# xcyan/neurips18_hierchical_image_manipulation

Hardware: AMD Instinct MI355X
Metric: mask2image train images/sec at 512x256 bs=8 (higher is better)
Workload: dtype f32; 1 GPU; C2: mask2image Cityscapes-shaped 512x256, GlobalGenerator ngf64/4down/9blocks (182.6M params) + 3-scale PatchGAN + VGG19 loss (synthetic weights), full train step G+D Adam, fp32; global_batch=8, per_gpu_batch=8, parallelism=dp1

## Files before the change

### include/him.h

```cpp
#ifndef HIM_H_
#define HIM_H_

#include <stddef.h>
#include <stdint.h>

#ifdef __cplusplus
extern "C" {
#endif

#define HIM_OK 0
#define HIM_E_INVALID (-1)
#define HIM_E_WORKSPACE (-2)
#define HIM_E_LAUNCH (-3)
#define HIM_E_UNSUPPORTED (-4)

#define HIM_ACT_NONE 0
#define HIM_ACT_RELU 1
#define HIM_ACT_LRELU 2
#define HIM_ACT_TANH 3
#define HIM_ACT_SIGMOID 4

#define HIM_PAD_ZERO 0
#define HIM_PAD_REFLECT 1

// ... 11 lines not shown
#define HIM_TILE_128x64 7

#define HIM_ALGO_NO_SPLITK (1u << 0)
#define HIM_ALGO_NO_DFOLD (1u << 1)
#define HIM_ALGO_WINO_PADDED_DGRAD (1u << 2)
#define HIM_ALGO_NO_SMALL_WIN (1u << 3)
#define HIM_ALGO_NO_FEWOUT_TILED (1u << 4)
#define HIM_ALGO_NO_FEWIN_TILED (1u << 5)
#define HIM_ALGO_NO_FEWCH_MFMA (1u << 6)
#define HIM_ALGO_GENERIC_CONV (1u << 7)
#define HIM_ALGO_NO_RESBLOCK_FUSED (1u << 8)
#define HIM_ALGO_NO_BGEMM (1u << 10)
#define HIM_ALGO_NO_ONEHOT_RLE (1u << 11)
#define HIM_ALGO_NO_FEWIN_FOLD (1u << 12)
#define HIM_ALGO_NO_FEWIN_REFLECT (1u << 14)
#define HIM_ALGO_NO_WINO_FUSED2 (1u << 15)
#define HIM_ALGO_NO_BGEMM_PERSISTENT (1u << 16)
#define HIM_ALGO_WINO4_TRAIN_FWD (1u << 13)
#define HIM_ALGO_FROZEN_WEIGHTS (1u << 9)

typedef struct HimAlgo {
  int wino_min_c;
  int wino_fused_min_c;
  int wino_fused_max_c;
  int wino4_min_c;
  int ksplit_max;
  int tile_wb, tile_nb;
  int wino_tblock;
  int wgrad_splits;
  unsigned disable;
  int wino_fused_chunk;
  int wgrad_tile;
} HimAlgo;
void him_algo_resolve(const HimAlgo* in, HimAlgo* out);
void him_algo_from_env(HimAlgo* a);

typedef struct HimConv2d {
  int B, Cin, H, W;
  int Cout, KH, KW;
  int stride, pad;
  int pad_mode;
  int OH, OW;
  int act;
  float slope;
  HimAlgo algo;
} HimConv2d;

size_t him_conv2d_fwd_ws(const HimConv2d* d);
int him_conv2d_fwd(const HimConv2d* d, const float* x, const float* w, const float* bias, float* y, void* ws,
                   size_t ws_bytes, void* stream);
size_t him_conv2d_bwd_data_ws(const HimConv2d* d);
int him_conv2d_bwd_data(const HimConv2d* d, const float* dy, const float* w, float* dx, void* ws,
                        size_t ws_bytes, void* stream);
size_t him_conv2d_bwd_weight_ws(const HimConv2d* d);
int him_conv2d_bwd_weight(const HimConv2d* d, const float* x, const float* dy, float* dw, float* dbias,
                          int accumulate, void* ws, size_t ws_bytes, void* stream);

typedef struct HimDeconv2d {
  int B, Cin, H, W;
  int Cout, KH, KW;
  int stride, pad, out_pad;
  int OH, OW;
  int act;
  float slope;
  HimAlgo algo;
} HimDeconv2d;
size_t him_deconv2d_fwd_ws(const HimDeconv2d* d);
int him_deconv2d_fwd(const HimDeconv2d* d, const float* x, const float* w, const float* bias, float* y,
                     void* ws, size_t ws_bytes, void* stream);
size_t him_deconv2d_bwd_data_ws(const HimDeconv2d* d);
int him_deconv2d_bwd_data(const HimDeconv2d* d, const float* dy, const float* w, float* dx, void* ws,
                          size_t ws_bytes, void* stream);
size_t him_deconv2d_bwd_weight_ws(const HimDeconv2d* d);
int him_deconv2d_bwd_weight(const HimDeconv2d* d, const float* x, const float* dy, float* dw, float* dbias,
                            int accumulate, void* ws, size_t ws_bytes, void* stream);
int him_conv2d_bwd_weight_plan(const HimConv2d* d, int* family, size_t* need_bytes, int* splits, int* tile_m, int* tile_n);
int him_deconv2d_bwd_weight_plan(const HimDeconv2d* d, int* family, size_t* need_bytes, int* splits, int* tile_m, int* tile_n);

size_t him_batchnorm_ws(int C);
int him_batchnorm_fwd(const float* x, const float* residual, const float* gamma, const float* beta, float* run_mean,
                      float* run_var, float* y, float* save_mean, float* save_rstd, int B, int C, int hw, float eps,
                      float momentum, int training, int act, float slope, void* ws, size_t ws_bytes, void* stream);
int him_batchnorm_bwd(const float* x, const float* gamma, const float* beta, const float* save_mean,
                      const float* save_rstd, const float* dy, float* dx, float* dgamma, float* dbeta, int B, int C,
                      int hw, int training, int act, float slope, int accumulate, void* ws, size_t ws_bytes,
                      void* stream);
int him_act_fwd(const float* x, float* y, size_t n, int act, float slope, void* stream);
int him_upsample2_fwd(const float* x, float* y, int planes, int H, int W, int align_corners, void* stream);
int him_upsample2_bwd(const float* dy, float* dx, int planes, int H, int W, int align_corners, void* stream);
int him_resize_compose(const float* comb_prob, const float* obj_prob, int C, int h, int w, const float* label,
                       const float* mask_out, int cls, int background, void* dst, int H, int W, int align_corners,
                       void* stream);
int him_logsoftmax_fwd(const float* x, float* y, int B, int C, int hw, void* stream);
int him_logsoftmax_bwd(const float* y, const float* dy, float* dx, int B, int C, int hw, void* stream);
int him_gate_comb_fwd(const float* ctx, const float* p, const float* obj, float* out, int B, int C, int hw, void* stream);
int him_gate_comb_bwd(const float* ctx, const float* p, const float* obj, const float* dout, float* dctx, float* dp,
                      float* dobj, int B, int C, int hw, void* stream);
size_t him_mask_loss_ws(void);
int him_masked_nll_fwd(const float* logp, const float* label, const float* mask, float* out2, int B, int C, int hw,
                       void* ws, size_t ws_bytes, void* stream);
int him_masked_nll_bwd(const float* label, const float* mask, const float* g, const float* count, float* dlogp, int B,
                       int C, int hw, void* stream);
int him_bce_mean_fwd(const float* p, const float* t, size_t n, float* out, void* ws, size_t ws_bytes, void* stream);
int him_bce_mean_bwd(const float* p, const float* t, size_t n, const float* g, float* dp, void* stream);
int him_space_to_batch(const float* x, float* y, int B, int C, int H, int W, int d, int inverse, void* stream);
int him_lr_control(const float* loss_d_real, const float* loss_d_fake, float margin, float* out2, void* stream);
int him_class_mask(const float* mask, const float* cls, float* dst, int B, int NC, int Ctot, int c0, int hw, void* stream);

size_t him_conv2d_onehot_fwd_ws(const HimConv2d* d, int n_onehot);
int him_conv2d_onehot_fwd(const HimConv2d* d, const float* label, int n_onehot, const float* x, const float* w,
// ... 258 lines not shown
```

### neurips18_hierchical_image_manipulation_amd/_cabi.py

```python
import ctypes as C
import os

_HERE = os.path.dirname(os.path.abspath(__file__))
LIB_PATH = os.path.join(_HERE, 'lib', 'libhim_hip.so')

c_float_p = C.c_void_p
c_int, c_size_t, c_float, c_void_p, c_double = C.c_int, C.c_size_t, C.c_float, C.c_void_p, C.c_double


class HimAlgo(C.Structure):
    _fields_ = [(n, c_int) for n in ('wino_min_c', 'wino_fused_min_c', 'wino_fused_max_c', 'wino4_min_c', 'ksplit_max',
                                     'tile_wb', 'tile_nb', 'wino_tblock', 'wgrad_splits')] + \
               [('disable', C.c_uint), ('wino_fused_chunk', c_int), ('wgrad_tile', c_int)]

    def as_dict(self):
        return {n: int(getattr(self, n)) for n, _ in self._fields_ if n != 'reserved'}


ALGO_NO_SPLITK, ALGO_NO_DFOLD, ALGO_WINO_PADDED_DGRAD, ALGO_NO_SMALL_WIN, ALGO_NO_FEWOUT_TILED, ALGO_NO_FEWIN_TILED, \
    ALGO_NO_FEWCH_MFMA, ALGO_GENERIC_CONV, ALGO_NO_RESBLOCK_FUSED, ALGO_FROZEN_WEIGHTS, ALGO_NO_BGEMM, ALGO_NO_ONEHOT_RLE = (1 << i for i in range(12))
ALGO_NO_FEWIN_FOLD = 1 << 12
ALGO_WINO4_TRAIN_FWD = 1 << 13
ALGO_NO_FEWIN_REFLECT = 1 << 14
ALGO_NO_WINO_FUSED2 = 1 << 15
ALGO_NO_BGEMM_PERSISTENT = 1 << 16
ONEHOT_PART_IDS, ONEHOT_PART_DENSE = 1, 2
TILE_DEFAULT, TILE_128x128, TILE_128x128_8W, TILE_128x256, TILE_64x128, TILE_64x64, TILE_MIXED, TILE_128x64 = range(8)


class HimConv2d(C.Structure):
    _fields_ = [(n, c_int) for n in ('B', 'Cin', 'H', 'W', 'Cout', 'KH', 'KW', 'stride', 'pad', 'pad_mode',
                                     'OH', 'OW', 'act')] + [('slope', c_float), ('algo', HimAlgo)]


class HimDeconv2d(C.Structure):
    _fields_ = [(n, c_int) for n in ('B', 'Cin', 'H', 'W', 'Cout', 'KH', 'KW', 'stride', 'pad', 'out_pad',
                                     'OH', 'OW', 'act')] + [('slope', c_float), ('algo', HimAlgo)]


class HimResBlock(C.Structure):
    _fields_ = [(n, c_int) for n in ('B', 'C', 'H', 'W')] + [('eps', c_float), ('algo', HimAlgo)]


ACT_NONE, ACT_RELU, ACT_LRELU, ACT_TANH, ACT_SIGMOID = 0, 1, 2, 3, 4
PAD_ZERO, PAD_REFLECT = 0, 1

P = c_void_p
_CONV, _DECONV, _RESB, _ALGO = C.POINTER(HimConv2d), C.POINTER(HimDeconv2d), C.POINTER(HimResBlock), C.POINTER(HimAlgo)

_SIGS = {
    'him_version': (C.c_char_p, []),
    'him_arch': (C.c_char_p, []),
    'him_last_error': (C.c_char_p, []),
    'him_conv2d_fwd_ws': (c_size_t, [_CONV]),
    'him_conv2d_fwd': (c_int, [_CONV, P, P, P, P, P, c_size_t, P]),
    'him_conv2d_bwd_data_ws': (c_size_t, [_CONV]),
    'him_conv2d_bwd_data': (c_int, [_CONV, P, P, P, P, c_size_t, P]),
    'him_conv2d_bwd_weight_ws': (c_size_t, [_CONV]),
    'him_conv2d_bwd_weight': (c_int, [_CONV, P, P, P, P, c_int, P, c_size_t, P]),
    'him_deconv2d_fwd_ws': (c_size_t, [_DECONV]),
    'him_deconv2d_fwd': (c_int, [_DECONV, P, P, P, P, P, c_size_t, P]),
    'him_deconv2d_bwd_data_ws': (c_size_t, [_DECONV]),
    'him_deconv2d_bwd_data': (c_int, [_DECONV, P, P, P, P, c_size_t, P]),
    'him_deconv2d_bwd_weight_ws': (c_size_t, [_DECONV]),
    'him_deconv2d_bwd_weight': (c_int, [_DECONV, P, P, P, P, c_int, P, c_size_t, P]),
    'him_conv2d_bwd_weight_plan': (c_int, [_CONV, C.POINTER(c_int), C.POINTER(c_size_t)] + [C.POINTER(c_int)] * 3),
    'him_deconv2d_bwd_weight_plan': (c_int, [_DECONV, C.POINTER(c_int), C.POINTER(c_size_t)] + [C.POINTER(c_int)] * 3),
    'him_algo_resolve': (None, [_ALGO, _ALGO]),
    'him_algo_from_env': (None, [_ALGO]),
    'him_conv2d_onehot_fwd_ws': (c_size_t, [_CONV, c_int]),
    'him_conv2d_onehot_fwd': (c_int, [_CONV, P, c_int, P, P, P, P, P, c_size_t, P]),
    'him_conv2d_onehot_bwd_weight_ws': (c_size_t, [_CONV, c_int]),
    'him_conv2d_onehot_bwd_weight': (c_int, [_CONV, P, c_int, P, P, P, P, c_int, P, c_size_t, P]),
    'him_conv2d_onehot_fwd_dense': (c_int, [_CONV, P, c_int, P, P, P, P, P, c_size_t, P]),
    'him_conv2d_onehot_bwd_weight_dense': (c_int, [_CONV, P, c_int, P, P, P, P, c_int, P, c_size_t, P]),
    'him_conv2d_onehot_bwd_weight_part': (c_int, [_CONV, P, c_int, P, c_int, P, P, P, c_int, P, c_size_t, c_int, P]),
    'him_winograd_gemm': (c_int, [P, P, P, c_int, c_int, c_int, _ALGO, P]),
    'him_conv2d_panel_bytes': (c_size_t, [_CONV, c_int]),
    'him_conv2d_bwd_data_shares_fwd_panel': (C.c_uint, [_CONV]),
    'him_conv2d_panel_layout': (C.c_uint, [_CONV, c_int]),
    'him_conv2d_panel_build': (c_int, [_CONV, c_int, P, P, c_size_t, P]),
    'him_conv2d_fwd_panel': (c_int, [_CONV, P, P, P, P, P, c_size_t, P]),
    'him_conv2d_bwd_data_panel': (c_int, [_CONV, P, P, P, P, c_size_t, P]),
    'him_conv2d_bwd_data_gated': (c_int, [_CONV, P, P, P, P, P, P, c_size_t, P]),
    'him_conv2d_fwd_keep_bytes': (c_size_t, [_CONV]),
    'him_conv2d_fwd_panel_keep': (c_int, [_CONV, P, P, P, P, P, P, c_size_t, P]),
    'him_conv2d_bwd_weight_kept': (c_int, [_CONV, P, P, P, P, c_int, P, c_size_t, P]),
    'him_deconv2d_panel_bytes': (c_size_t, [_DECONV, c_int]),
    'him_deconv2d_panel_build': (c_int, [_DECONV, c_int, P, P, c_size_t, P]),
    'him_deconv2d_fwd_panel': (c_int, [_DECONV, P, P, P, P, P, c_size_t, P]),
    'him_deconv2d_bwd_data_panel': (c_int, [_DECONV, P, P, P, P, c_size_t, P]),
    'him_batchnorm_ws': (c_size_t, [c_int]),
    'him_batchnorm_fwd': (c_int, [P, P, P, P, P, P, P, P, P, c_int, c_int, c_int, c_float, c_float, c_int, c_int, c_float,
                                  P, c_size_t, P]),
    'him_batchnorm_bwd': (c_int, [P, P, P, P, P, P, P, P, P, c_int, c_int, c_int, c_int, c_int, c_float, c_int, P,
                                  c_size_t, P]),
    'him_act_fwd': (c_int, [P, P, c_size_t, c_int, c_float, P]),
    'him_upsample2_fwd': (c_int, [P, P, c_int, c_int, c_int, c_int, P]),
    'him_upsample2_bwd': (c_int, [P, P, c_int, c_int, c_int, c_int, P]),
    'him_resize_compose': (c_int, [P, P, c_int, c_int, c_int, P, P, c_int, c_int, P, c_int, c_int, c_int, P]),
# ... 164 lines not shown
```

### neurips18_hierchical_image_manipulation_amd/csrc/him_conv.hip

```cpp
#include <stdlib.h>

#include <algorithm>
#include <type_traits>

#include "him_common.h"

namespace him {

#include "him_gconv_fast.inc"
#include "him_wino_fused.inc"
#include "him_wino_fused2.inc"
#include "him_bgemm.inc"

struct WT2Phase {
  float* out;
  int JH, JW;
  long long sh, sw, base;
  long long total;
};
struct WT2P {
  const float* W;
  int M, C2, C2p;
  long long sm, sc;
  WT2Phase ph[4];
// ... 402 lines not shown
  if (reflect) hipLaunchKernelGGL((wino_input_kernel<true>), gin, dim3(tb), 0, st, src, V, gi);
  else hipLaunchKernelGGL((wino_input_kernel<false>), gin, dim3(tb), 0, st, src, V, gi);
  int rc = check_launch("wino_input");
  if (rc) return rc;
  rc = wino_batched_gemm(a, U, V, Mo, Mout, Csrc, gi.Tp, st, atrans);
  if (rc) return rc;
  WinoGeom go = gi;
  go.C = Mout;
  hipLaunchKernelGGL(wino_output_kernel, dim3(cdiv(gi.Tp, tb), Mout), dim3(tb), 0, st, (const float*)Mo, dst, bias, go,
                     act, slope);
  return check_launch("wino_output");
}

#include "him_conv_wino4.inc"

#include "him_conv_wgrad.inc"

#include "him_wgrad_fewch.inc"

enum WGradFamily { WGRAD_WINO, WGRAD_HEAD, WGRAD_STEM, WGRAD_SMALL_WIN, WGRAD_SMALL, WGRAD_FAST, WGRAD_GENERIC };
struct WGradShape {
  int M, C, B, H, W, OH, OW, KH, KW, stride, pad, pad_mode;
  int Np() const { return C * KH * KW; }
  int Kdim() const { return B * OH * OW; }
};
static WGradShape wgrad_shape(const HimConv2d* d) {
  return {d->Cout, d->Cin, d->B, d->H, d->W, d->OH, d->OW, d->KH, d->KW, d->stride, d->pad, d->pad_mode};
}
struct WGradPlan {
  HimAlgo algo;
  WGradShape s;
  WGradFamily family;
  int BM, BN;
  int splits;
  int kchunk;
  bool reduce;
  size_t need_bytes;
  size_t slab_bytes;
};
static const int SMALL_WIN_SLOTS = 256;
static int small_wgrad_slices(int C, int Kdim) {
  int s = (2048 + C - 1) / C;
  const int maxs = cdiv(Kdim, 256 * 8);
  if (s > maxs) s = maxs;
  return s < 1 ? 1 : s;
}
static bool small_win_class(int M, int KH, int KW) { return M <= 4 && KH == KW && (KH == 3 || KH == 5 || KH == 7); }
static bool small_class(int M, int KH, int KW) { return M <= 4 && KH == KW && (KH == 7 || KH == 4 || KH == 3); }
static bool wgrad_same_geom(const WGradShape& s) {
  return s.stride == 1 && s.pad == s.KH / 2 && s.OH == s.H && s.OW == s.W && s.H > s.pad && s.W > s.pad;
}
static size_t round256(size_t n) { return (n + 255) / 256 * 256; }

static WGradPlan plan_wgrad(const HimAlgo& a, const WGradShape& s, bool allow_wino) {
  WGradPlan p;
  memset(&p, 0, sizeof(p));
  p.algo = a;
  p.s = s;
  p.splits = 1;
  p.reduce = true;
  const int M = s.M, C = s.C, Kdim = s.Kdim();
  const auto slabs = [&](int n) { return (size_t)n * M * s.Np() * sizeof(float); };
  const bool head_c = fewch_class(a, M, C, s.KH, s.KW), stem_c = fewch_class(a, C, M, s.KH, s.KW);
  const bool win_c = small_win_class(M, s.KH, s.KW), small_c = small_class(M, s.KH, s.KW), fast_c = wgrad_fast_class(a, M, C);
  const int fewch_tc = head_c ? C : M, slices = small_wgrad_slices(C, Kdim), tiny_n = std::max(slices, SMALL_WIN_SLOTS);
  int gBM, gBN, fBM = 0, fBN = 0, fs = 0;
  wgrad_tile(M, &gBM, &gBN);
  int gs = wgrad_splits(M, s.Np(), Kdim, gBM, gBN);
  if (win_c && !small_c && !head_c) gs = std::min(gs, tiny_n);
  if (fast_c) wgrad_fast_cfg(a, M, C, Kdim, s.KH * s.KW, &fBM, &fBN, &fs);
  const size_t generic = gs > 1 ? slabs(gs) : 0, tiny = slabs(tiny_n);
  const bool fits31 = (unsigned long long)s.B * M * s.OH * s.OW * 4ull < (1ull << 31) &&
                      (unsigned long long)s.B * C * s.H * s.W * 4ull < (1ull << 31);
  if (allow_wino && wino_wgrad_ok(a, M, C, s.KH, s.KW, s.stride, s.pad, s.H, s.W) && s.OH == s.H && s.OW == s.W) {
    p.family = WGRAD_WINO;
    p.need_bytes = wino_wgrad_floats(s.B, M, C, s.OH, s.OW) * sizeof(float);
    p.slab_bytes = round256(p.need_bytes);
    return p;
  }
  if ((head_c || stem_c) && wgrad_same_geom(s)) {
    p.family = head_c ? WGRAD_HEAD : WGRAD_STEM;
    p.splits = std::min(fewch_geom(head_c, s.B, s.H, s.W, s.pad).ntask, FEWCH_WGS);
    p.need_bytes = fewch_need_bytes(fewch_tc, s.KH, p.splits);
  } else if (win_c && !algo_off(a, HIM_ALGO_NO_SMALL_WIN) && wgrad_same_geom(s)) {
    p.family = WGRAD_SMALL_WIN;
    p.splits = std::min(s.B * cdiv(s.W, 64) * cdiv(s.H, 64), SMALL_WIN_SLOTS);
    p.need_bytes = slabs(p.splits);
  } else if (small_c) {
    p.family = WGRAD_SMALL;
    p.splits = slices;
    p.kchunk = cdiv(Kdim, slices);
    p.need_bytes = slabs(slices);
  } else if (fast_c && s.OH * s.OW >= 4 && fits31) {
    p.family = WGRAD_FAST;
    p.BM = fBM, p.BN = fBN, p.splits = fs;
    p.kchunk = (cdiv(Kdim, fs) + 31) / 32 * 32;
    p.need_bytes = slabs(fs);
  } else {
    p.family = WGRAD_GENERIC;
    p.BM = gBM, p.BN = gBN, p.splits = gs;
    p.kchunk = (cdiv(Kdim, gs) + 31) / 32 * 32;
    p.reduce = gs > 1;
    p.need_bytes = generic;
  }
  size_t b;
  if (head_c || stem_c) b = std::max(std::max(fewch_need_bytes(fewch_tc, s.KH, FEWCH_WGS), generic), (win_c || small_c) ? tiny : 0);
  else if (win_c || small_c) b = tiny;
  else if (fast_c) b = std::max(slabs(fs), generic);
  else b = generic;
  p.slab_bytes = round256(b);
  return p;
}

static int wgrad_finish(const WGradPlan& p, const char* what, const float* part, float* dw, int accumulate, hipStream_t st) {
  const int rc = check_launch(what);
  if (rc || !p.reduce) return rc;
  if (p.family == WGRAD_FAST) {
    hipLaunchKernelGGL(wgrad_finish_kernel, dim3(p.s.C / 64, p.s.M), dim3(256), 0, st, part, dw, p.s.M, p.s.C, p.s.KH * p.s.KW,
                       p.splits, accumulate);
    return check_launch("wgrad_finish");
  }
  const long long n = (long long)p.s.M * p.s.Np();
  hipLaunchKernelGGL(slab_reduce_kernel, dim3(std::min<long long>(cdiv(n, 256), 4096)), dim3(256), 0, st, part, dw, n, p.splits,
                     accumulate);
  return check_launch("slab_reduce");
}

static int run_wgrad(const WGradPlan& pl, const float* dy, const float* x, float* dw, int accumulate, void* ws, size_t ws_bytes,
                     hipStream_t st, const float* kept_v = nullptr) {
  if (pl.need_bytes && (ws_bytes < pl.need_bytes || !ws))
// ... 45 lines not shown
    case WGRAD_HEAD:
    case WGRAD_STEM:
      return run_wgrad_fewch(pl.family == WGRAD_HEAD, dy, x, dw, M, C, B, H, W, KH, s.pad, s.pad_mode, pl.splits, accumulate, ws, st);
    case WGRAD_SMALL_WIN: {
      const int nsx = cdiv(W, 64), rows_per = 64, nyc = cdiv(H, rows_per), ntasks = B * nsx * nyc;
      const dim3 grid(pl.splits, cdiv(C, 4));
#define HIM_SWK(MMv, KSv)                                                                                         \
  if (M == MMv && KH == KSv) {                                                                                    \
    constexpr int TRv = (MMv * KSv * KSv > 90) ? (KSv + 1) / 2 : KSv;   \
    const dim3 gridz(grid.x, grid.y, cdiv(KSv, TRv));                                                             \
    if (refl) hipLaunchKernelGGL((wgrad_small_win_kernel<MMv, KSv, TRv, true>), gridz, block, 0, st, p, nsx, nyc, rows_per, ntasks); \
    else hipLaunchKernelGGL((wgrad_small_win_kernel<MMv, KSv, TRv, false>), gridz, block, 0, st, p, nsx, nyc, rows_per, ntasks);     \
  }
      HIM_SWK(1, 3) HIM_SWK(2, 3) HIM_SWK(3, 3) HIM_SWK(4, 3)
      HIM_SWK(1, 5) HIM_SWK(2, 5) HIM_SWK(3, 5) HIM_SWK(4, 5)
      HIM_SWK(1, 7) HIM_SWK(2, 7) HIM_SWK(3, 7) HIM_SWK(4, 7)
#undef HIM_SWK
      return wgrad_finish(pl, "wgrad_small_win", (const float*)ws, dw, accumulate, st);
    }
    case WGRAD_SMALL: {
      const dim3 grid(C, pl.splits);
#define HIM_WS(MMv, TJv)                                                                             \
  if (M == MMv && KH == TJv) {                                                                       \
    if (refl) hipLaunchKernelGGL((wgrad_small_kernel<MMv, TJv, true>), grid, block, 0, st, p);        \
    else hipLaunchKernelGGL((wgrad_small_kernel<MMv, TJv, false>), grid, block, 0, st, p);            \
  }
      HIM_WS(1, 7) HIM_WS(2, 7) HIM_WS(3, 7) HIM_WS(4, 7)
      HIM_WS(1, 4) HIM_WS(2, 4) HIM_WS(3, 4) HIM_WS(4, 4)
      HIM_WS(1, 3) HIM_WS(2, 3) HIM_WS(3, 3) HIM_WS(4, 3)
#undef HIM_WS
      return wgrad_finish(pl, "wgrad_small", (const float*)ws, dw, accumulate, st);
    }
    case WGRAD_FAST: {
      const dim3 grid(p.Np / pl.BN, cdiv(M, pl.BM), pl.splits);
#define HIM_WF(TMv, TNv)                                                                              \
  {                                                                                                   \
    if ((s.OH * s.OW) % 4 == 0) {                                                                     \
      if (refl) hipLaunchKernelGGL((wgrad_fast_kernel<TMv, TNv, true, true>), grid, block, 0, st, p);  \
      else hipLaunchKernelGGL((wgrad_fast_kernel<TMv, TNv, false, true>), grid, block, 0, st, p);      \
    } else {                                                                                          \
      if (refl) hipLaunchKernelGGL((wgrad_fast_kernel<TMv, TNv, true, false>), grid, block, 0, st, p); \
      else hipLaunchKernelGGL((wgrad_fast_kernel<TMv, TNv, false, false>), grid, block, 0, st, p);     \
    }                                                                                                 \
  }
      if (pl.BM == 128 && pl.BN == 128) HIM_WF(2, 2)
      else if (pl.BM == 128) HIM_WF(2, 1)
      else if (pl.BN == 128) HIM_WF(1, 2)
      else HIM_WF(1, 1)
#undef HIM_WF
      return wgrad_finish(pl, "wgrad_fast", (const float*)ws, dw, accumulate, st);
    }
    case WGRAD_GENERIC: {
      const dim3 grid(cdiv(p.Np, pl.BN), cdiv(M, pl.BM), pl.splits);
      if (pl.BM == 128) {
        if (refl) hipLaunchKernelGGL((wgrad_kernel<2, 2, 2, 2, true>), grid, block, 0, st, p);
        else hipLaunchKernelGGL((wgrad_kernel<2, 2, 2, 2, false>), grid, block, 0, st, p);
      } else if (pl.BM == 64) {
        if (refl) hipLaunchKernelGGL((wgrad_kernel<1, 4, 2, 1, true>), grid, block, 0, st, p);
        else hipLaunchKernelGGL((wgrad_kernel<1, 4, 2, 1, false>), grid, block, 0, st, p);
      } else {
        if (refl) hipLaunchKernelGGL((wgrad_kernel<1, 4, 1, 1, true>), grid, block, 0, st, p);
        else hipLaunchKernelGGL((wgrad_kernel<1, 4, 1, 1, false>), grid, block, 0, st, p);
      }
      return wgrad_finish(pl, "wgrad", (const float*)ws, dw, accumulate, st);
    }
  }
// ... 501 lines not shown
  c->OH = t->H;
  c->OW = t->W;
  c->act = HIM_ACT_NONE;
  c->slope = 0.f;
  c->algo = t->algo;
  if ((c->H + 2 * c->pad - c->KH) / c->stride + 1 != c->OH || (c->W + 2 * c->pad - c->KW) / c->stride + 1 != c->OW)
    return fail(HIM_E_UNSUPPORTED, "deconv2d: output_padding %d not representable", t->out_pad);
  return check_conv(c);
}

}

using namespace him;

#include "him_resblock.inc"

extern "C" {

void him_algo_resolve(const HimAlgo* in, HimAlgo* out) {
  if (!out) return;
  HimAlgo z;
  memset(&z, 0, sizeof(z));
  const HimAlgo& a = in ? *in : z;
  HimAlgo r = a;
  r.wino_min_c = algo_wino_min_c(a);
  r.wino_fused_min_c = algo_wino_fused_min_c(a);
  r.wino_fused_max_c = algo_wino_fused_max_c(a);
  r.wino4_min_c = algo_wino4_min_c(a);
  r.ksplit_max = algo_off(a, HIM_ALGO_NO_SPLITK) ? 1 : algo_ksplit_max(a);
  r.tile_wb = a.tile_wb == HIM_TILE_DEFAULT ? HIM_TILE_64x128 : a.tile_wb;
  r.tile_nb = a.tile_nb == HIM_TILE_DEFAULT ? HIM_TILE_64x128 : a.tile_nb;
  r.wino_tblock = algo_tblock(a);
  r.wino_fused_chunk = algo_wino_fused_chunk(a);
  r.wgrad_tile = (a.wgrad_tile == 1 || a.wgrad_tile == 2) ? a.wgrad_tile : 0;
  *out = r;
}

void him_algo_from_env(HimAlgo* a) {
  if (!a) return;
  memset(a, 0, sizeof(*a));
  auto geti = [](const char* k, int dflt) { const char* e = getenv(k); return e ? atoi(e) : dflt; };
  a->wino_min_c = getenv("HIM_NO_WINOGRAD") ? -1 : geti("HIM_WINO_MIN_C", 0);
  a->wino_fused_min_c = getenv("HIM_NO_WINO_FUSED") ? -1 : geti("HIM_WINO_FUSED_MIN_C", 0);
  a->wino_fused_max_c = geti("HIM_WINO_FUSED_MAX_C", 0);
  a->wino4_min_c = getenv("HIM_NO_WINO4") ? -1 : geti("HIM_WINO4_MIN_C", 0);
  a->ksplit_max = geti("HIM_KSPLIT_MAX", 0);
  const int tile_all = geti("HIM_GCONV_TILE", 0);
  a->tile_wb = geti("HIM_GCONV_TILE_WB", tile_all);
  a->tile_nb = geti("HIM_GCONV_TILE_NB", tile_all);
  a->wino_tblock = geti("HIM_WINO_TBLOCK", 0);
  a->wgrad_splits = geti("HIM_WGRAD_SPLITS", 0);
  a->wino_fused_chunk = geti("HIM_WINO_FUSED_CHUNK", 0);
  a->wgrad_tile = geti("HIM_WGRAD_TILE", 0);
  const struct { const char* k; unsigned bit; } flags[] = {
      {"HIM_NO_SPLITK", HIM_ALGO_NO_SPLITK},           {"HIM_NO_DFOLD", HIM_ALGO_NO_DFOLD},
      {"HIM_WINO_PADDED_DGRAD", HIM_ALGO_WINO_PADDED_DGRAD}, {"HIM_NO_SMALL_WIN", HIM_ALGO_NO_SMALL_WIN},
      {"HIM_NO_FEWOUT_TILED", HIM_ALGO_NO_FEWOUT_TILED}, {"HIM_NO_FEWIN_TILED", HIM_ALGO_NO_FEWIN_TILED},
      {"HIM_NO_FEWCH_MFMA", HIM_ALGO_NO_FEWCH_MFMA},   {"HIM_GENERIC_CONV", HIM_ALGO_GENERIC_CONV},
      {"HIM_NO_RESBLOCK_FUSED", HIM_ALGO_NO_RESBLOCK_FUSED}, {"HIM_NO_BGEMM", HIM_ALGO_NO_BGEMM},
      {"HIM_NO_ONEHOT_RLE", HIM_ALGO_NO_ONEHOT_RLE},   {"HIM_NO_FEWIN_FOLD", HIM_ALGO_NO_FEWIN_FOLD},
      {"HIM_WINO4_TRAIN_FWD", HIM_ALGO_WINO4_TRAIN_FWD}, {"HIM_NO_FEWIN_REFLECT", HIM_ALGO_NO_FEWIN_REFLECT},
      {"HIM_NO_WINO_FUSED2", HIM_ALGO_NO_WINO_FUSED2}, {"HIM_NO_BGEMM_PERSISTENT", HIM_ALGO_NO_BGEMM_PERSISTENT}};
  for (const auto& f : flags)
    if (getenv(f.k)) a->disable |= f.bit;
}

int him_winograd_gemm(const float* a, const float* b, float* c, int M, int K, int N, const HimAlgo* algo, void* stream) {
  if (!a || !b || !c || M <= 4 || K < 16 || (K % 16) || N <= 0 || (N % 128))
    return fail(HIM_E_INVALID, "winograd gemm: need M > 4, K %% 16 == 0, N %% 128 == 0 (got %d, %d, %d)", M, K, N);
  if ((long long)16 * K * N >= (1ll << 31) || (long long)16 * M * N >= (1ll << 31))
    return fail(HIM_E_UNSUPPORTED, "winograd gemm: operand larger than 2^31 elements");
  HimAlgo z;
  memset(&z, 0, sizeof(z));
  return wino_batched_gemm(algo ? *algo : z, a, b, c, M, K, N, (hipStream_t)stream);
}

size_t him_conv2d_fwd_ws(const HimConv2d* d) { return d ? plan_fprop(d).ws_bytes : 0; }

int him_conv2d_fwd(const HimConv2d* d, const float* x, const float* w, const float* bias, float* y, void* ws,
                   size_t ws_bytes, void* stream) {
  int rc = check_conv(d);
  if (rc) return rc;
  return run_fprop(d, x, w, bias, y, ws, ws_bytes, (hipStream_t)stream);
}

int him_conv2d_in_act_fused(const HimConv2d* d) { return (d && !check_conv(d) && plan_fprop(d).in_act_slab) ? 1 : 0; }
// ... 106 lines not shown
}
static int conv_bwd_weight(const HimConv2d* d, const float* x, const float* keep, const float* dy, float* dw, float* dbias,
                           int accumulate, void* ws, size_t ws_bytes, hipStream_t st) {
  const WGradPlan p = plan_wgrad(d->algo, wgrad_shape(d), true);
  if (dw) {
    int rc = run_wgrad(p, dy, x, dw, accumulate, ws, ws_bytes, st, keep);
    if (rc) return rc;
  }
  if (!dbias) return HIM_OK;
  return run_bias_grad_behind(dy, dbias, d->B, d->Cout, d->OH * d->OW, accumulate, ws, ws_bytes, p.slab_bytes, st);
}
int him_conv2d_bwd_weight_kept(const HimConv2d* d, const float* keep, const float* dy, float* dw, float* dbias, int accumulate,
                               void* ws, size_t ws_bytes, void* stream) {
  int rc = check_conv(d);
  if (rc) return rc;
  if (!keep || !fwd_keep_ok(d)) return fail(HIM_E_INVALID, "conv bwd_weight_kept: no kept transform for this descriptor");
  return conv_bwd_weight(d, nullptr, keep, dy, dw, dbias, accumulate, ws, ws_bytes, (hipStream_t)stream);
}

size_t him_conv2d_bwd_weight_ws(const HimConv2d* d) {
  return d ? plan_wgrad(d->algo, wgrad_shape(d), true).slab_bytes + bias_ws_bytes(d->Cout) : 0;
}
static int report_wgrad_plan(const WGradPlan& p, int* family, size_t* need_bytes, int* splits, int* tile_m, int* tile_n) {
  if (family) *family = p.family;
  if (need_bytes) *need_bytes = p.need_bytes;
  if (splits) *splits = p.splits;
  if (tile_m) *tile_m = p.BM;
  if (tile_n) *tile_n = p.BN;
  return HIM_OK;
}
int him_conv2d_bwd_weight_plan(const HimConv2d* d, int* family, size_t* need_bytes, int* splits, int* tile_m, int* tile_n) {
  const int rc = check_conv(d);
  return rc ? rc : report_wgrad_plan(plan_wgrad(d->algo, wgrad_shape(d), true), family, need_bytes, splits, tile_m, tile_n);
}

int him_conv2d_bwd_weight(const HimConv2d* d, const float* x, const float* dy, float* dw, float* dbias,
                          int accumulate, void* ws, size_t ws_bytes, void* stream) {
  int rc = check_conv(d);
  if (rc) return rc;
  return conv_bwd_weight(d, x, nullptr, dy, dw, dbias, accumulate, ws, ws_bytes, (hipStream_t)stream);
}

size_t him_conv2d_onehot_fwd_ws(const HimConv2d* d, int n_onehot) {
  return (d && !check_conv(d) && onehot_ok(d, n_onehot)) ? onehot_fwd_ws_bytes(d, n_onehot) : 0;
}

static int onehot_fwd_impl(const HimConv2d* d, const float* label, int n_onehot, const float* x, bool x_dense, const float* w,
                           const float* bias, float* y, void* ws, size_t ws_bytes, void* stream) {
  int rc = check_conv(d);
  if (rc) return rc;
  if (!onehot_ok(d, n_onehot))
    return fail(HIM_E_UNSUPPORTED, "onehot conv: needs an odd 'same' stride-1 kernel or 4x4 stride 2 zero-padded, Cout %% 16 == 0");
  if (!ws || ws_bytes < onehot_fwd_ws_bytes(d, n_onehot)) return fail(HIM_E_WORKSPACE, "onehot conv fwd: ws too small");
  hipStream_t st = (hipStream_t)stream;
  const int NC = n_onehot, Cd = d->Cin - NC, KK = d->KH * d->KW, HW = d->H * d->W;
  float* Wt = (float*)ws;
  float* xd = Wt + ((size_t)KK * NC * d->Cout + 63) / 64 * 64;
  hipLaunchKernelGGL(onehot_table_kernel, dim3(cdiv((long long)KK * NC * d->Cout, 256)), dim3(256), 0, st, w, Wt, d->Cout,
                     d->Cin, NC, KK);
  if (Cd > 0) {
    float* wd = xd + ((size_t)d->B * Cd * HW + 63) / 64 * 64;
    float* cws = wd + ((size_t)d->Cout * Cd * KK + 63) / 64 * 64;
    if (!x_dense) {
      rc = him_copy_channels(x, d->Cin, NC, xd, Cd, 0, Cd, d->B, HW, nullptr, 0, 0, stream);
      if (rc) return rc;
    }
// ... 192 lines not shown
  return him_conv2d_panel_build(&c, kind == HIM_PANEL_FWD ? HIM_PANEL_BWD_DATA : HIM_PANEL_FWD, w, panel, panel_bytes,
                                stream);
}

int him_deconv2d_fwd_panel(const HimDeconv2d* t, const float* x, const void* panel, const float* bias, float* y,
                           void* ws, size_t ws_bytes, void* stream) {
  HimConv2d c;
  int rc = adjoint_of(t, &c);
  if (rc) return rc;
  if (!panel) return fail(HIM_E_INVALID, "deconv fwd: null panel");
  return run_dgrad(&c, x, nullptr, y, bias, t->act, t->slope, ws, ws_bytes, (hipStream_t)stream, (const float*)panel);
}

int him_deconv2d_bwd_data_panel(const HimDeconv2d* t, const float* dy, const void* panel, float* dx, void* ws,
                                size_t ws_bytes, void* stream) {
  HimConv2d c;
  int rc = adjoint_of(t, &c);
  if (rc) return rc;
  if (!panel || !plan_fprop(&c).panel_floats) return fail(HIM_E_INVALID, "deconv bwd_data: no panel for this descriptor");
  return run_fprop(&c, dy, nullptr, nullptr, dx, ws, ws_bytes, (hipStream_t)stream, (const float*)panel);
}

size_t him_deconv2d_bwd_weight_ws(const HimDeconv2d* t) {
  HimConv2d c;
  if (adjoint_of(t, &c)) return 0;
  return plan_wgrad(c.algo, wgrad_shape(&c), false).slab_bytes + bias_ws_bytes(t->Cout);
}
int him_deconv2d_bwd_weight_plan(const HimDeconv2d* t, int* family, size_t* need_bytes, int* splits, int* tile_m, int* tile_n) {
  HimConv2d c;
  const int rc = adjoint_of(t, &c);
  return rc ? rc : report_wgrad_plan(plan_wgrad(c.algo, wgrad_shape(&c), false), family, need_bytes, splits, tile_m, tile_n);
}

int him_deconv2d_bwd_weight(const HimDeconv2d* t, const float* x, const float* dy, float* dw, float* dbias,
                            int accumulate, void* ws, size_t ws_bytes, void* stream) {
  HimConv2d c;
  int rc = adjoint_of(t, &c);
  if (rc) return rc;
  const WGradPlan p = plan_wgrad(c.algo, wgrad_shape(&c), false);
  if (dw) {
    rc = run_wgrad(p, x, dy, dw, accumulate, ws, ws_bytes, (hipStream_t)stream);
    if (rc) return rc;
  }
  if (!dbias) return HIM_OK;
  return run_bias_grad_behind(dy, dbias, t->B, t->Cout, t->OH * t->OW, accumulate, ws, ws_bytes, p.slab_bytes, (hipStream_t)stream);
}

}
```

### neurips18_hierchical_image_manipulation_amd/csrc/him_conv_wgrad.inc

```
struct WGradP {
  const float* dy;
  const float* x;
  float* out;
  int M, C, B, H, W, OH, OW, KH, KW, stride, pad, pad_mode;
  int Np, Kdim, kchunk, splits, accumulate;
  FastDiv fKK, fKW, fOW;
};

template <int WM, int WN, int TM, int TN, bool REFLECT>
__global__ __launch_bounds__(256) void wgrad_kernel(const WGradP p) {
  constexpr int BM = WM * TM * 32, BN = WN * TN * 32, BK = 32;
  constexpr int LD = BK + 1;
  constexpr int RA = BM / 8, RB = BN / 8;
  static_assert(WM * WN == 4, "4 waves");
  __shared__ float sA[2][BM * LD];
  __shared__ float sB[2][BN * LD];
  __shared__ int tabOff[BN];
  __shared__ int tabD[BN];

  const int t = threadIdx.x, lane = t & 63, wave = t >> 6;
  const int wm = wave / WN, wn = wave % WN;
  const int n0 = blockIdx.x * BN, m0 = blockIdx.y * BM;
  const int OHW = p.OH * p.OW, HW = p.H * p.W;
  const int kbeg = blockIdx.z * p.kchunk;
// ... 310 lines not shown
      __builtin_amdgcn_sched_group_barrier(0x200, A_V4 + RB, 0);                                              \
      __builtin_amdgcn_sched_group_barrier(0x008, 6, 0);                                                      \
    }                                                                                                         \
    __syncthreads();                                                                                          \
  }
  {
    int kt = 0;
    for (; kt + 1 < nk; kt += 2) {
      HIM_WKSTEP(kt, raX, rbX, raY, rbY)
      HIM_WKSTEP(kt + 1, raY, rbY, raX, rbX)
    }
    if (kt < nk) HIM_WKSTEP(kt, raX, rbX, raY, rbY)
  }
#undef HIM_WKSTEP
#undef HIM_WM
#undef HIM_WLOAD
#undef HIM_WSTORE

  float* __restrict__ out = p.out + (size_t)blockIdx.z * p.M * p.Np;
#pragma unroll
  for (int j = 0; j < TN; ++j) {
    const int np = n0 + wn * TN * 32 + j * 32 + l31;
#pragma unroll
    for (int i = 0; i < TM; ++i) {
#pragma unroll
      for (int r = 0; r < 16; ++r) {
        const int m = m0 + wm * TM * 32 + i * 32 + (r & 3) + 8 * (r >> 2) + 4 * lh;
        if (m < p.M) out[(size_t)m * p.Np + np] = acc[i][j][r];
      }
    }
  }
}

__global__ __launch_bounds__(256) void wgrad_finish_kernel(const float* __restrict__ slabs, float* __restrict__ dw,
                                                           int M, int C, int KK, int splits, int accumulate) {
  __shared__ float sm[64 * 49];
  const int m = blockIdx.y, c0 = blockIdx.x * 64;
  const size_t n = (size_t)M * C * KK;
  const int nel = 64 * KK;
  for (int i = threadIdx.x; i < nel; i += 256) {
    const int tap = i >> 6, ci = i & 63;
    const size_t src = (size_t)m * C * KK + (size_t)tap * C + c0 + ci;
    float v = 0.f;
    for (int z = 0; z < splits; ++z) v += slabs[(size_t)z * n + src];
    sm[ci * KK + tap] = v;
  }
  __syncthreads();
  float* __restrict__ dst = dw + ((size_t)m * C + c0) * KK;
  for (int i = threadIdx.x; i < nel; i += 256) dst[i] = accumulate ? dst[i] + sm[i] : sm[i];
}

static bool wgrad_fast_class(const HimAlgo& a, int M, int C) { return !algo_off(a, HIM_ALGO_GENERIC_CONV) && M > 4 && (C % 64) == 0; }
static void wgrad_fast_cfg(const HimAlgo& a, int M, int C, int Kdim, int KK, int* BM, int* BN, int* splits) {
  *BM = (M > 64 && a.wgrad_tile == 0) ? 128 : 64;
  *BN = ((C % 128) == 0 && a.wgrad_tile != 2) ? 128 : 64;
  const long long tiles = (long long)cdiv(M, *BM) * ((long long)C * KK / *BN);
  int s = (int)((768 + tiles - 1) / tiles);
  const int maxs = cdiv(Kdim, 32 * 8);
  if (s > maxs) s = maxs;
  if (s < 1) s = 1;
  if (s > 256) s = 256;
  if (a.wgrad_splits > 0) s = std::max(1, std::min(maxs, a.wgrad_splits));
  *splits = s;
}

template <int MM, int TJ, bool REFLECT>
__global__ __launch_bounds__(256) void wgrad_small_kernel(const WGradP p) {
  __shared__ float red[4][MM * TJ * TJ];
  const int c = blockIdx.x;
  const int t = threadIdx.x;
  const int OHW = p.OH * p.OW, HW = p.H * p.W;
  const int kbeg = blockIdx.y * p.kchunk;
  const int kend = min(p.Kdim, kbeg + p.kchunk);
  float acc[MM][TJ][TJ];
#pragma unroll
  for (int m = 0; m < MM; ++m)
#pragma unroll
    for (int a = 0; a < TJ; ++a)
#pragma unroll
      for (int b2 = 0; b2 < TJ; ++b2) acc[m][a][b2] = 0.f;
  const int H = p.H, W = p.W;
  for (int k = kbeg + t; k < kend; k += 256) {
    const int b = k / OHW;
    const int sp = k - b * OHW;
    const int oh = (int)fdiv((uint32_t)sp, p.fOW);
    const int ow = sp - oh * p.OW;
    float g[MM];
#pragma unroll
// ... 241 lines not shown
```

Measured before the change: 160.2 images/s.

## Add tap-row wgrad kernel for stride-2 3x3 zero-pad convolutions

Adds a specialized weight-gradient kernel for 3x3 stride-2 pad-1 convs that processes one kernel row of taps per block. It loads each input row once as float2 pairs plus a halo element and scatters them into three tap columns in shared memory, so one staged load serves all three horizontal taps instead of gathering each im2col column separately. It uses buffer loads, double buffering and explicit MFMA/load scheduling barriers. It adds edge-case logic for the halo and row boundaries, so correctness depends on intricate indexing; an env switch can disable it.

```diff
diff --git a/include/him.h b/include/him.h
--- a/include/him.h
+++ b/include/him.h
@@ -67,6 +67,7 @@
   int wino_fused_chunk;
   int wgrad_tile;
 } HimAlgo;
+#define HIM_WGRAD_TILE_NO_TAPROW 4
 void him_algo_resolve(const HimAlgo* in, HimAlgo* out);
 void him_algo_from_env(HimAlgo* a);
 
@@ -111,6 +112,8 @@
                             int accumulate, void* ws, size_t ws_bytes, void* stream);
 int him_conv2d_bwd_weight_plan(const HimConv2d* d, int* family, size_t* need_bytes, int* splits, int* tile_m, int* tile_n);
 int him_deconv2d_bwd_weight_plan(const HimDeconv2d* d, int* family, size_t* need_bytes, int* splits, int* tile_m, int* tile_n);
+int him_conv2d_bwd_weight_taprow(const HimConv2d* d);
+int him_deconv2d_bwd_weight_taprow(const HimDeconv2d* d);
 
 size_t him_batchnorm_ws(int C);
 int him_batchnorm_fwd(const float* x, const float* residual, const float* gamma, const float* beta, float* run_mean,
diff --git a/neurips18_hierchical_image_manipulation_amd/_cabi.py b/neurips18_hierchical_image_manipulation_amd/_cabi.py
--- a/neurips18_hierchical_image_manipulation_amd/_cabi.py
+++ b/neurips18_hierchical_image_manipulation_amd/_cabi.py
@@ -24,6 +24,7 @@
 ALGO_NO_FEWIN_REFLECT = 1 << 14
 ALGO_NO_WINO_FUSED2 = 1 << 15
 ALGO_NO_BGEMM_PERSISTENT = 1 << 16
+WGRAD_TILE_NO_TAPROW = 4
 ONEHOT_PART_IDS, ONEHOT_PART_DENSE = 1, 2
 TILE_DEFAULT, TILE_128x128, TILE_128x128_8W, TILE_128x256, TILE_64x128, TILE_64x64, TILE_MIXED, TILE_128x64 = range(8)
 
@@ -66,6 +67,8 @@
     'him_deconv2d_bwd_weight': (c_int, [_DECONV, P, P, P, P, c_int, P, c_size_t, P]),
     'him_conv2d_bwd_weight_plan': (c_int, [_CONV, C.POINTER(c_int), C.POINTER(c_size_t)] + [C.POINTER(c_int)] * 3),
     'him_deconv2d_bwd_weight_plan': (c_int, [_DECONV, C.POINTER(c_int), C.POINTER(c_size_t)] + [C.POINTER(c_int)] * 3),
+    'him_conv2d_bwd_weight_taprow': (C.c_uint, [_CONV]),
+    'him_deconv2d_bwd_weight_taprow': (C.c_uint, [_DECONV]),
     'him_algo_resolve': (None, [_ALGO, _ALGO]),
     'him_algo_from_env': (None, [_ALGO]),
     'him_conv2d_onehot_fwd_ws': (c_size_t, [_CONV, c_int]),
diff --git a/neurips18_hierchical_image_manipulation_amd/csrc/him_conv.hip b/neurips18_hierchical_image_manipulation_amd/csrc/him_conv.hip
--- a/neurips18_hierchical_image_manipulation_amd/csrc/him_conv.hip
+++ b/neurips18_hierchical_image_manipulation_amd/csrc/him_conv.hip
@@ -458,6 +458,7 @@
   WGradShape s;
   WGradFamily family;
   int BM, BN;
+  bool taprow;
   int splits;
   int kchunk;
   bool reduce;
@@ -522,6 +523,8 @@
     p.BM = fBM, p.BN = fBN, p.splits = fs;
     p.kchunk = (cdiv(Kdim, fs) + 31) / 32 * 32;
     p.need_bytes = slabs(fs);
+    p.taprow = !(a.wgrad_tile & HIM_WGRAD_TILE_NO_TAPROW) && s.KH == 3 && s.KW == 3 && s.stride == 2 && s.pad == 1 &&
+               s.pad_mode == HIM_PAD_ZERO && (s.W % 2) == 0 && s.OW * 2 == s.W && (s.OH * s.OW) % 4 == 0;
   } else {
     p.family = WGRAD_GENERIC;
     p.BM = gBM, p.BN = gBN, p.splits = gs;
@@ -633,6 +636,12 @@
       return wgrad_finish(pl, "wgrad_small", (const float*)ws, dw, accumulate, st);
     }
     case WGRAD_FAST: {
+      if (pl.taprow && ((uintptr_t)x & 7) == 0) {
+        const dim3 gridt(3 * (C / 32), cdiv(M, pl.BM), pl.splits);
+        if (pl.BM == 128) hipLaunchKernelGGL((wgrad_taprow_kernel<4>), gridt, dim3(256), 0, st, p);
+        else hipLaunchKernelGGL((wgrad_taprow_kernel<2>), gridt, dim3(128), 0, st, p);
+        return wgrad_finish(pl, "wgrad_taprow", (const float*)ws, dw, accumulate, st);
+      }
       const dim3 grid(p.Np / pl.BN, cdiv(M, pl.BM), pl.splits);
 #define HIM_WF(TMv, TNv)                                                                              \
   {                                                                                                   \
@@ -1200,7 +1209,8 @@
   r.tile_nb = a.tile_nb == HIM_TILE_DEFAULT ? HIM_TILE_64x128 : a.tile_nb;
   r.wino_tblock = algo_tblock(a);
   r.wino_fused_chunk = algo_wino_fused_chunk(a);
-  r.wgrad_tile = (a.wgrad_tile == 1 || a.wgrad_tile == 2) ? a.wgrad_tile : 0;
+  const int wt = a.wgrad_tile & ~HIM_WGRAD_TILE_NO_TAPROW;
+  r.wgrad_tile = ((wt == 1 || wt == 2) ? wt : 0) | (a.wgrad_tile & HIM_WGRAD_TILE_NO_TAPROW);
   *out = r;
 }
 
@@ -1219,7 +1229,7 @@
   a->wino_tblock = geti("HIM_WINO_TBLOCK", 0);
   a->wgrad_splits = geti("HIM_WGRAD_SPLITS", 0);
   a->wino_fused_chunk = geti("HIM_WINO_FUSED_CHUNK", 0);
-  a->wgrad_tile = geti("HIM_WGRAD_TILE", 0);
+  a->wgrad_tile = geti("HIM_WGRAD_TILE", 0) | (getenv("HIM_NO_WGRAD_TAPROW") ? HIM_WGRAD_TILE_NO_TAPROW : 0);
   const struct { const char* k; unsigned bit; } flags[] = {
       {"HIM_NO_SPLITK", HIM_ALGO_NO_SPLITK},           {"HIM_NO_DFOLD", HIM_ALGO_NO_DFOLD},
       {"HIM_WINO_PADDED_DGRAD", HIM_ALGO_WINO_PADDED_DGRAD}, {"HIM_NO_SMALL_WIN", HIM_ALGO_NO_SMALL_WIN},
@@ -1392,6 +1402,10 @@
 int him_conv2d_bwd_weight_plan(const HimConv2d* d, int* family, size_t* need_bytes, int* splits, int* tile_m, int* tile_n) {
   const int rc = check_conv(d);
   return rc ? rc : report_wgrad_plan(plan_wgrad(d->algo, wgrad_shape(d), true), family, need_bytes, splits, tile_m, tile_n);
+}
+
+int him_conv2d_bwd_weight_taprow(const HimConv2d* d) {
+  return (d && !check_conv(d) && plan_wgrad(d->algo, wgrad_shape(d), true).taprow) ? 1 : 0;
 }
 
 int him_conv2d_bwd_weight(const HimConv2d* d, const float* x, const float* dy, float* dw, float* dbias,
@@ -1650,6 +1664,11 @@
   return rc ? rc : report_wgrad_plan(plan_wgrad(c.algo, wgrad_shape(&c), false), family, need_bytes, splits, tile_m, tile_n);
 }
 
+int him_deconv2d_bwd_weight_taprow(const HimDeconv2d* t) {
+  HimConv2d c;
+  return (!adjoint_of(t, &c) && plan_wgrad(c.algo, wgrad_shape(&c), false).taprow) ? 1 : 0;
+}
+
 int him_deconv2d_bwd_weight(const HimDeconv2d* t, const float* x, const float* dy, float* dw, float* dbias,
                             int accumulate, void* ws, size_t ws_bytes, void* stream) {
   HimConv2d c;
diff --git a/neurips18_hierchical_image_manipulation_amd/csrc/him_conv_wgrad.inc b/neurips18_hierchical_image_manipulation_amd/csrc/him_conv_wgrad.inc
--- a/neurips18_hierchical_image_manipulation_amd/csrc/him_conv_wgrad.inc
+++ b/neurips18_hierchical_image_manipulation_amd/csrc/him_conv_wgrad.inc
@@ -366,6 +366,188 @@
   }
 }
 
+template <int NW>
+__global__ __launch_bounds__(64 * NW) void wgrad_taprow_kernel(const WGradP p) {
+  constexpr int NT = 64 * NW, BM = 32 * NW, CB = 32, BK = 32, LD = 36;
+  constexpr int A_V4 = 4;
+  constexpr int AR = NT / 8;
+  constexpr int NRG = NT / 32, CPT = CB / NRG;
+  constexpr int DUMP = 3 * CB * LD;
+  __shared__ __attribute__((aligned(16))) float sA[2][BM * LD];
+  __shared__ __attribute__((aligned(16))) float sB[2][4 * CB * LD];
+
+  const int t = threadIdx.x, lane = t & 63, wave = t >> 6;
+  const int OHW = p.OH * p.OW, HW = p.H * p.W, C = p.C;
+  const int kbeg = blockIdx.z * p.kchunk;
+  const int kend = min(p.Kdim, kbeg + p.kchunk);
+  const int nk = (kend - kbeg + BK - 1) / BK;
+  const int ncb = C / CB;
+  const int th = blockIdx.x / ncb, ci0 = (blockIdx.x - th * ncb) * CB;
+  const int m0 = blockIdx.y * BM;
+  const int H = p.H, W = p.W, OWm1 = p.OW - 1;
+
+  const int arow = t >> 3, akq = t & 7;
+  uint32_t arowoff[A_V4];
+#pragma unroll
+  for (int i = 0; i < A_V4; ++i) arowoff[i] = (uint32_t)min(m0 + arow + AR * i, p.M - 1) * (uint32_t)OHW;
+  const int kkl = t & 31, rg = t >> 5;
+
+  const __amdgpu_buffer_rsrc_t rdy = __builtin_amdgcn_make_buffer_rsrc(
+      (void*)p.dy, 0, (int)((uint32_t)p.B * (uint32_t)p.M * (uint32_t)OHW * 4u), 0x00020000);
+  const __amdgpu_buffer_rsrc_t rx = __builtin_amdgcn_make_buffer_rsrc(
+      (void*)p.x, 0, (int)((uint32_t)p.B * (uint32_t)C * (uint32_t)HW * 4u), 0x00020000);
+  const uint32_t xbase = (uint32_t)ci0 * (uint32_t)HW * 4u;
+  const uint32_t stepg = (uint32_t)NRG * (uint32_t)HW * 4u;
+
+  float4 raX[A_V4], raY[A_V4];
+  float2 rbX[CPT], rbY[CPT];
+  float rzX[CPT], rzY[CPT];
+  int wnX, wnY, woX, woY;
+  int ka = kbeg + akq * 4, ba = ka / OHW, spa = ka - ba * OHW;
+  int kb = kbeg + kkl, bb = kb / OHW, spb = kb - bb * OHW;
+
+#define HIM_TLOAD(ra, rb, rz, wn, wo)                                                                          \
+  {                                                                                                           \
+    if (HIM_WG_DBG & 2) {                                                                                     \
+      _Pragma("unroll") for (int i = 0; i < A_V4; ++i) ra[i] = make_float4(1.f, 1.f, 1.f, 1.f);               \
+    } else {                                                                                                  \
+      const bool av = ka < kend;                                                                              \
+      const uint32_t abase = (uint32_t)ba * (uint32_t)p.M * (uint32_t)OHW + (uint32_t)spa;                     \
+      _Pragma("unroll") for (int i = 0; i < A_V4; ++i) {                                                      \
+        ra[i] = __builtin_bit_cast(                                                                            \
+            float4, __builtin_amdgcn_raw_buffer_load_b128(rdy, av ? (abase + arowoff[i]) * 4u : 0x80000000u, 0, 0)); \
+      }                                                                                                       \
+    }                                                                                                         \
+    const bool bv = kb < kend;                                                                                \
+    const int sp = bv ? spb : 0;                                                                              \
+    const int oh = (int)fdiv((uint32_t)sp, p.fOW);                                                            \
+    const int ow = sp - oh * p.OW;                                                                            \
+    const int ih = 2 * oh + th - 1;                                                                           \
+    const bool ok = bv && ih >= 0 && ih < H;                                                                  \
+    const uint32_t voff = ok ? ((uint32_t)bb * (uint32_t)C * (uint32_t)HW + (uint32_t)rg * (uint32_t)HW +      \
+                                (uint32_t)ih * (uint32_t)W + 2u * (uint32_t)ow) * 4u : 0x80000000u;            \
+    const uint32_t voff0 = (ok && kkl == 0 && ow > 0) ? voff - 4u : 0x80000000u;                               \
+     \
+    wn = ((kkl < BK - 1 && ow != OWm1 && kb + 1 < kend) ? 0 : DUMP) + rg * LD + kkl + 1;                       \
+    wo = ((kkl == 0 || ow == 0) ? 0 : DUMP) + rg * LD + kkl;               \
+    uint32_t so = xbase;                                                                                      \
+    _Pragma("unroll") for (int i = 0; i < CPT; ++i) {                                                         \
+      if (HIM_WG_DBG & 1) {                                                                                   \
+        rb[i] = make_float2(__builtin_bit_cast(float, voff), __builtin_bit_cast(float, so));                  \
+        rz[i] = __builtin_bit_cast(float, voff0);                                                             \
+      } else {                                                                                                \
+        rb[i] = __builtin_bit_cast(float2, __builtin_amdgcn_raw_buffer_load_b64(rx, voff, so, 0));            \
+        rz[i] = __builtin_bit_cast(float, __builtin_amdgcn_raw_buffer_load_b32(rx, voff0, so, 0));            \
+      }                                                                                                       \
+      so += stepg;                                                                                            \
+    }                                                                                                         \
+    ka += BK;                                                                                                 \
+    spa += BK;                                                                                                \
+    while (spa >= OHW) {                                                                                      \
+      spa -= OHW;                                                                                             \
+      ++ba;                                                                                                   \
+    }                                                                                                         \
+    kb += BK;                                                                                                 \
+    spb += BK;                                                                                                \
+    while (spb >= OHW) {                                                                                      \
+      spb -= OHW;                                                                                             \
+      ++bb;                                                                                                   \
+    }                                                                                                         \
+  }
+#define HIM_TSTORE(buf_, ra, rb, rz, wn, wo)                                                                   \
+  if (!(HIM_WG_DBG & 4)) {                                                                                    \
+    _Pragma("unroll") for (int i = 0; i < A_V4; ++i) *(float4*)&sA[buf_][(arow + AR * i) * LD + akq * 4] = ra[i]; \
+    _Pragma("unroll") for (int i = 0; i < CPT; ++i) {                                                         \
+      float* __restrict__ r_ = &sB[buf_][NRG * i * LD];                                                       \
+      r_[(CB + rg) * LD + kkl] = rb[i].x;                                                                     \
+      r_[(2 * CB + rg) * LD + kkl] = rb[i].y;                                                                 \
+      r_[wn] = rb[i].y;                                                                                       \
+      r_[wo] = rz[i];                                                                                         \
+    }                                                                                                         \
+  } else {                                                                                                    \
+    float sink_ = 0.f;                                                                                        \
+    _Pragma("unroll") for (int i = 0; i < A_V4; ++i) sink_ += ra[i].x + ra[i].y + ra[i].z + ra[i].w;          \
+    _Pragma("unroll") for (int i = 0; i < CPT; ++i) sink_ += rb[i].x + rb[i].y + rz[i];                       \
+    if (sink_ == 1.2345e-30f) sB[buf_][(wn + wo) & 1] = sink_;                                                \
+  }
+
+  f32x16 acc[3];
+#pragma unroll
+  for (int j = 0; j < 3; ++j)
+#pragma unroll
+    for (int r = 0; r < 16; ++r) acc[j][r] = 0.f;
+
+  const int l31 = lane & 31, lh = lane >> 5;
+  if (nk > 0) {
+    HIM_TLOAD(raX, rbX, rzX, wnX, woX)
+    HIM_TSTORE(0, raX, rbX, rzX, wnX, woX)
+    HIM_TLOAD(raY, rbY, rzY, wnY, woY)
+  }
+  __syncthreads();
+#define HIM_TM(Q, CMP)                                                                                         \
+  _Pragma("unroll") for (int j = 0; j < 3; ++j) {                                                              \
+    if (HIM_WG_DBG & 8) acc[j][0] += af[Q].CMP * bf[j][Q].CMP;                                                \
+    else acc[j] = __builtin_amdgcn_mfma_f32_32x32x2f32(af[Q].CMP, bf[j][Q].CMP, acc[j], 0, 0, 0);             \
+  }
+#define HIM_TKSTEP(kt_, LA, LB, LZ, LN, LO, SA, SB, SZ, SN, SO)                                                 \
+  {                                                                                                           \
+    const int buf = (kt_) & 1;                                                                                \
+    const float4* __restrict__ pa = (const float4*)&sA[buf][(wave * 32 + l31) * LD + lh * 16];                \
+    const float4* __restrict__ pb = (const float4*)&sB[buf][l31 * LD + lh * 16];                              \
+    float4 af[4], bf[3][4];                                                                                   \
+_Pragma("unroll")                                                                                             \
+    for (int q = 0; q < 4; ++q) af[q] = pa[q];                                                                \
+_Pragma("unroll")                                                                                             \
+    for (int j = 0; j < 3; ++j)                                                                               \
+_Pragma("unroll")                                                                                             \
+      for (int q = 0; q < 4; ++q) bf[j][q] = pb[j * CB * LD / 4 + q];                                         \
+    HIM_TLOAD(LA, LB, LZ, LN, LO)          \
+    HIM_TM(0, x) HIM_TM(0, y) HIM_TM(0, z) HIM_TM(0, w)                                                       \
+    HIM_TM(1, x) HIM_TM(1, y) HIM_TM(1, z) HIM_TM(1, w)                                                       \
+    HIM_TM(2, x) HIM_TM(2, y) HIM_TM(2, z) HIM_TM(2, w)                                                       \
+    HIM_TM(3, x) HIM_TM(3, y) HIM_TM(3, z) HIM_TM(3, w)                                                       \
+    HIM_TSTORE(buf ^ 1, SA, SB, SZ, SN, SO)                                                                   \
+    {                                                                                                         \
+       \
+      constexpr int NV = A_V4 + 2 * CPT, NM = 48, PER = (NM - 10) / NV;                                       \
+      __builtin_amdgcn_sched_group_barrier(0x100, 16, 0);                                                     \
+      __builtin_amdgcn_sched_group_barrier(0x008, 2, 0);                                                      \
+_Pragma("unroll")                                                                                             \
+      for (int q_ = 0; q_ < NV; ++q_) {                                                                       \
+        __builtin_amdgcn_sched_group_barrier(0x020, 1, 0);                                                    \
+        __builtin_amdgcn_sched_group_barrier(0x008, PER, 0);                                                  \
+      }                                                                                                       \
+      __builtin_amdgcn_sched_group_barrier(0x008, NM - 2 - PER * NV - 6, 0);                                  \
+      __builtin_amdgcn_sched_group_barrier(0x200, A_V4 + 4 * CPT, 0);                                         \
+      __builtin_amdgcn_sched_group_barrier(0x008, 6, 0);                                                      \
+    }                                                                                                         \
+    __syncthreads();                                                                                          \
+  }
+  {
+    int kt = 0;
+    for (; kt + 1 < nk; kt += 2) {
+      HIM_TKSTEP(kt, raX, rbX, rzX, wnX, woX, raY, rbY, rzY, wnY, woY)
+      HIM_TKSTEP(kt + 1, raY, rbY, rzY, wnY, woY, raX, rbX, rzX, wnX, woX)
+    }
+    if (kt < nk) HIM_TKSTEP(kt, raX, rbX, rzX, wnX, woX, raY, rbY, rzY, wnY, woY)
+  }
+#undef HIM_TKSTEP
+#undef HIM_TM
+#undef HIM_TLOAD
+#undef HIM_TSTORE
+
+  float* __restrict__ out = p.out + (size_t)blockIdx.z * p.M * p.Np;
+#pragma unroll
+  for (int j = 0; j < 3; ++j) {
+    const int np = (th * 3 + j) * C + ci0 + l31;
+#pragma unroll
+    for (int r = 0; r < 16; ++r) {
+      const int m = m0 + wave * 32 + (r & 3) + 8 * (r >> 2) + 4 * lh;
+      if (m < p.M) out[(size_t)m * p.Np + np] = acc[j][r];
+    }
+  }
+}
+
 __global__ __launch_bounds__(256) void wgrad_finish_kernel(const float* __restrict__ slabs, float* __restrict__ dw,
                                                            int M, int C, int KK, int splits, int accumulate) {
   __shared__ float sm[64 * 49];
@@ -386,8 +568,9 @@
 
 static bool wgrad_fast_class(const HimAlgo& a, int M, int C) { return !algo_off(a, HIM_ALGO_GENERIC_CONV) && M > 4 && (C % 64) == 0; }
 static void wgrad_fast_cfg(const HimAlgo& a, int M, int C, int Kdim, int KK, int* BM, int* BN, int* splits) {
-  *BM = (M > 64 && a.wgrad_tile == 0) ? 128 : 64;
-  *BN = ((C % 128) == 0 && a.wgrad_tile != 2) ? 128 : 64;
+  const int tile = a.wgrad_tile & ~HIM_WGRAD_TILE_NO_TAPROW;
+  *BM = (M > 64 && tile == 0) ? 128 : 64;
+  *BN = ((C % 128) == 0 && tile != 2) ? 128 : 64;
   const long long tiles = (long long)cdiv(M, *BM) * ((long long)C * KK / *BN);
   int s = (int)((768 + tiles - 1) / tiles);
   const int maxs = cdiv(Kdim, 32 * 8);
```

After: 160.7 images/s, median of 6. Within noise of the previous version (+0.3%).
